# dusk-network/plonk

Measured on AMD Instinct MI355X. Metric: prove() wall-clock (ms) at 2^20 gates, lower is better.
Workload: dtype u32 limbs (Fr 256-bit / Fp 384-bit Montgomery)

## Files before the change

### plonk_amd/__init__.py

```python
from __future__ import annotations

import ctypes
import os
import weakref
from typing import Iterable, Sequence

os.environ.setdefault("HSA_ENABLE_IPC_MODE_LEGACY", "0")

_HERE = os.path.dirname(os.path.abspath(__file__))
LIB_PATH = os.environ.get("PLONK_HIP_LIB") or os.path.join(_HERE, "lib", "libplonk_hip.so")

Q = 0x73EDA753299D7D483339D80809A1D80553BDA402FFFE5BFEFFFFFFFF00000001
P = 0x1A0111EA397FE69A4B1BA7B6434BACD764774B84F38512BF6730D2A0F6B0F6241EABFFFEB153FFFFB9FEFFFFFFFFAAAB
_FR_R = (1 << 256) % Q
_FR_RINV = pow(_FR_R, -1, Q)
_FP_R = (1 << 384) % P
_FP_RINV = pow(_FP_R, -1, P)

PLONK_OK = 0
ERRORS = {
    -1: "PLONK_ERR_ARG", -2: "PLONK_ERR_HIP", -3: "PLONK_ERR_DEGREE (PolynomialDegreeTooLarge)",
    -4: "PLONK_ERR_NO_SRS", -5: "PLONK_ERR_NO_GPU", -6: "PLONK_ERR_UNSAT (CircuitUnsatisfied)",
    -7: "PLONK_ERR_STATE", -8: "PLONK_ERR_BYTES (NotEnoughBytes)", -9: "PLONK_ERR_DATA (InvalidData)",
    -10: "PLONK_ERR_POINT (PointMalformed)", -11: "PLONK_ERR_NOMEM (host allocation failed inside the library)",
# ... 260 lines not shown
    lib.plonk_srs_load_public_parameters.argtypes = [vp, vp, u64, u64, ci, vp, ctypes.POINTER(u64)]
    lib.plonk_lagrange_key.argtypes = [vp, u32, vp]
    lib.plonk_compile.argtypes = [vp, ctypes.POINTER(_CircuitDesc), ctypes.POINTER(vp)]
    lib.plonk_prover_prove_witnesses.argtypes = [vp, vp, u64, vp, vp, u64, vp, vp]
    lib.plonk_prover_to_bytes.argtypes = [vp, vp, u64, ctypes.POINTER(u64)]
    lib.plonk_verifier_to_bytes.argtypes = [vp, vp, u64, vp, u64, vp, u64, ctypes.POINTER(u64)]
    lib.plonk_verifier_from_bytes.argtypes = [vp, vp, u64, ctypes.POINTER(vp)]
    lib.plonk_verifier_destroy.argtypes = [vp]
    lib.plonk_verifier_destroy.restype = None
    lib.plonk_verifier_set_version.argtypes = [vp, ci]
    lib.plonk_verify.argtypes = [vp, vp, vp, u64, u64, vp]
    lib.plonk_verifier_last.argtypes = [vp, vp]
    lib.plonk_test_verify_msm.argtypes = [vp, vp, vp, u64, vp]
    lib.plonk_verify_mixed.argtypes = [vp, u32, vp, vp, vp, u64, u64, vp, vp]
    lib.plonk_test_verify_replay.argtypes = [vp, u32, vp, vp, vp, u64, u64, vp, vp, vp]
    lib.plonk_host_alloc.argtypes = [u64, ctypes.POINTER(vp)]
    lib.plonk_host_free.argtypes = [vp]
    lib.plonk_comm_unique_id.argtypes = [vp]
    lib.plonk_comm_init.argtypes = [vp, vp, ci, ci]
    lib.plonk_comm_selftest.argtypes = [vp]
    lib.plonk_comm_info.argtypes = [vp, ctypes.POINTER(ci), ctypes.POINTER(ci)]
    lib.plonk_comm_destroy.argtypes = [vp]
    lib.plonk_comm_warning.argtypes = [vp, vp, u64]
    lib.plonk_comm_measure_loopback.argtypes = [vp, ci]
    lib.plonk_ctx_create_ex.argtypes = [ctypes.POINTER(vp), ci, ctypes.POINTER(GpuConfig)]
    lib.plonk_ctx_get_config.argtypes = [vp, ctypes.POINTER(GpuConfig)]
    lib.plonk_ctx_set_config.argtypes = [vp, ctypes.POINTER(GpuConfig)]
    lib.plonk_ctx_describe_msm.argtypes = [vp, u64, ci, ci, u32, u64, ctypes.POINTER(_MsmPlan)]
    lib.plonk_ctx_last_msm.argtypes = [vp, ctypes.POINTER(_MsmPlan)]
    lib.plonk_ctx_table_bytes.argtypes = [vp, ctypes.POINTER(u64), ctypes.POINTER(u64)]
# ... 284 lines not shown
        out = ctypes.create_string_buffer(97)
        self._check(self.lib.plonk_test_verify_msm(self.handle, comp, sc, len(points), out))
        return g1_from_raw97(out.raw)

    def _verify_replay(self, items):
        args = _mixed_args(items)
        count = len(items)
        status = (ctypes.c_int32 * count)()
        scalars = ctypes.create_string_buffer(28 * 32 * count)
        digests = ctypes.create_string_buffer(32 * count)
        self._check(self.lib.plonk_test_verify_replay(*args, status, scalars, digests))
        raw = scalars.raw
        return [(int(status[k]), [raw[896 * k + 32 * j:896 * k + 32 * j + 32] for j in range(28)],
                 digests.raw[32 * k:32 * k + 32]) for k in range(count)]

    def alloc(self, nbytes: int) -> DeviceBuffer:
        return DeviceBuffer(self, nbytes)

    def get_config(self) -> "GpuConfig":
        g = GpuConfig()
        self._check(self.lib.plonk_ctx_get_config(self.handle, ctypes.byref(g)))
        return g

    def set_config(self, config: "GpuConfig"):
        self._check(self.lib.plonk_ctx_set_config(self.handle, ctypes.byref(config)))

    def describe_msm(self, m: int, count: int = 1, bit_sum_tail: bool = True, table_rows: int = 0, table_points: int = 0) -> dict:
        p = _MsmPlan()
        self._check(self.lib.plonk_ctx_describe_msm(self.handle, m, count, int(bit_sum_tail), table_rows, table_points, ctypes.byref(p)))
        return p.as_dict()
# ... 685 lines not shown
```

### plonk_amd/csrc/capi.hip

```cpp
#include <chrono>
#include <cstdio>
#include <cstring>
#include <sched.h>
#include <thread>

#include "plonk_internal.hpp"
#include "hostg1.hpp"

namespace plonk {

static thread_local char g_last_error[512] = "";

void set_last_error(const char* what, const char* detail, const char* file, int line) {
  snprintf(g_last_error, sizeof g_last_error, "%s:%d: %s -> %s", file, line, what ? what : "?", detail ? detail : "?");
}

int srs_generate_device(Ctx* c, const Fr& tau, const Fr& g_scalar, uint64_t n, G1Affine* out_dev);

int ctx_refuse_poisoned(const char* api_fn) {
  set_last_error(api_fn, "context unusable: a collective timed out and its stream never drained (comm_sync); destroy the context", __FILE__, __LINE__);
  return PLONK_ERR_STATE;
}

bool ctx_abandon(Ctx* c) {
// ... 171 lines not shown
  if (const int t = env_int("PLONK_COMM_TIMEOUT_MS", 0); t > 0) g.comm_timeout_ms = t;
  if (getenv("PLONK_SIDE_CUS")) g.side_cus = env_int("PLONK_SIDE_CUS", 0);
  g.ksl = env_int("PLONK_MSM_KSL", 0);
  g.prof_fine = env_chr("PLONK_PROF_FINE") == '1';
  g.acc_lds = env_chr("PLONK_MSM_ACC") == 'l';
  if (const char v = env_chr("PLONK_MSM_ORDER")) g.order = v == '1' ? 1 : 0;
  g.tail_serial = env_chr("PLONK_MSM_TAIL") == 's';
  g.bsum_lane = env_chr("PLONK_MSM_BSUM") == 'l';
  g.rc_lane_tree = env_chr("PLONK_MSM_RCTREE") == 'l';
  g.lps = env_int("PLONK_MSM_LPS", 0);
  g.rcwv = env_int("PLONK_MSM_RCWV", 0);
  if (const char v = env_chr("PLONK_MSM_SORT13")) g.sort13 = v == '1' ? 1 : 0;
  g.acc_wg = env_int("PLONK_MSM_ACC_WG", 0);
  g.ntt_direct = env_chr("PLONK_NTT_DIRECT") != '0';
  g.bi_cfg = env_int("PLONK_BI_CFG", -1);
  if (const char v = env_chr("PLONK_SIDE_DEFER")) g.side_defer = v == '1' ? 1 : (v == '2' ? 2 : 0);
  if (const char v = env_chr("PLONK_SIDE_AFTER_ELOG"); v == '2' || v == '3') g.side_after_elog = v - '0';
  if (const char v = env_chr("PLONK_WIRE_POLYS_SIDE")) g.wire_polys_side = v == '1' ? 1 : 0;
  if (env_chr("PLONK_WIRE_BY_COLUMN") == '0') g.wire_by_column = -1;
  if (env_chr("PLONK_WIRE_BY_COLUMN") == '1') g.wire_by_column = 1;
  if (env_chr("PLONK_WIRE_BY_COLUMN") == '2') g.wire_by_column = 2;
  if (getenv("PLONK_HOST_THREADS")) g.host_threads = env_int("PLONK_HOST_THREADS", -1);
  if (g.table_mode != (int)MSM_ROWS_WINDOW && g.table_mode != (int)MSM_ROWS_HALFPOS && g.table_mode != (int)MSM_ROWS_BITPOS) g.table_mode = 0;
  if (g.ntt_elog != 2 && g.ntt_elog != 3) g.ntt_elog = 0;
  if (g.side_cus < 0) g.side_cus = 0;
  if (g.host_threads < 0) {
    cpu_set_t set;
    CPU_ZERO(&set);
    const int cpus = sched_getaffinity(0, sizeof set, &set) == 0 ? CPU_COUNT(&set) : (int)std::thread::hardware_concurrency();
    g.host_threads = cpus >= 8 ? 3 : 0;
// ... 266 lines not shown
  return PLONK_OK;
  });
}

int plonk_ntt_dev(plonk_ctx* ctx, const void* src, void* dst, void* tmp, uint32_t log_n, int inverse,
                  int coset, uint64_t in_len) {
  const char* const api_fn = __func__;
  return plonk::api_guard(api_fn, [&]() -> int {
  if (!ctx || !src || !dst || log_n >= 28) return PLONK_ERR_ARG;
  if (log_n > 10 && !tmp) return PLONK_ERR_ARG;
  CTX_ENTER(ctx->c, api_fn);
  HIP_TRY(hipSetDevice(ctx->c.device));
  prof_begin(&ctx->c, 0);
  int rc = ntt_device(&ctx->c, (const Fr*)src, (Fr*)dst, (Fr*)tmp, log_n, inverse != 0, coset != 0, in_len);
  prof_end(&ctx->c, 0);
  return rc;
  });
}

int plonk_ntt(plonk_ctx* ctx, uint64_t* a, uint32_t log_n, int inverse, int coset, uint64_t in_len) {
  const char* const api_fn = __func__;
  return plonk::api_guard(api_fn, [&]() -> int {
  if (!ctx || !a || log_n >= 28) return PLONK_ERR_ARG;
  Ctx& c = ctx->c;
  CTX_ENTER(c, api_fn);
  HIP_TRY(hipSetDevice(c.device));
  const uint64_t n = 1ull << log_n;
  if (in_len > n) in_len = n;
  int rc = ensure_ntt_staging(&c, n);
  if (rc) return rc;
// ... 299 lines not shown
```

### plonk_amd/csrc/kzg.hip

```cpp
#include <hip/hip_runtime.h>

#include <chrono>
#include <memory>
#include <mutex>
#include <new>
#include <vector>

#include "../../include/plonk_hip.h"
#include "plonk_internal.hpp"
#include "api_guard.hpp"
#include "poly.hpp"
#include "fr29.cuh"
#include "hostg1.hpp"
#include "hostpairing.hpp"
#include "verify_core.hpp"
#include "kzg_core.hpp"

#define PTRY_K(expr) do { int _rc = (expr); if (_rc) return _rc; } while (0)
#define KZG_FAIL(code, msg) return (plonk::set_last_error(api_fn, msg, __FILE__, __LINE__), code)

namespace plonk { struct KzgKey; }
struct plonk_kzg_key {
  plonk::KzgKey* k;
  plonk_ctx* ctx;
// ... 148 lines not shown
  for (uint32_t i = 0; i < n; ++i) L = desc[i].len > L ? desc[i].len : L;
  if (L > c.srs_n) return PLONK_ERR_DEGREE;
  identity48(witness48);
  if (!L) {
    for (uint64_t i = 0; i < 4 * count; ++i) evaluations[i] = 0;
    if (commitments) for (uint32_t i = 0; i < n; ++i) identity48(commitments + 48ull * i);
    return PLONK_OK;
  }
  PTRY_K(msm_reserve(&c, L));
  PTRY_K(w.need(KzgWork::DESC, sizeof(KzgDesc) * n));
  PTRY_K(w.need(KzgWork::VPOW, sizeof(Fr29Slot) * n));
  PTRY_K(w.need(KzgWork::EVALS, sizeof(Fr) * n));
  PTRY_K(w.need(KzgWork::PARTIAL, sizeof(Fr) * KZG_GROUP * kzg_fold_waves(L)));
  PTRY_K(w.need(KzgWork::FOLD, sizeof(Fr) * (L + 1)));
  PTRY_K(w.need(KzgWork::SCRATCH, sizeof(Fr) * (L + 1)));
  PTRY_K(w.need(KzgWork::TOTALS, sizeof(Fr) * (L / 2048 + 2)));
  prof_begin(&c, 12);
  PTRY_K(poly_kzg_powers(&c, w.p[KzgWork::VPOW], n, v));
  HIP_TRY(hipMemsetAsync(w.p[KzgWork::EVALS], 0, sizeof(Fr) * n, c.stream));
  bool started = false;
  if (resident) {
    for (uint32_t first = 0; first < n; first += KZG_GROUP) {
      const uint32_t cnt = n - first < KZG_GROUP ? n - first : KZG_GROUP;
      uint64_t glen = 0;
      for (uint32_t i = 0; i < cnt; ++i) glen = desc[first + i].len > glen ? desc[first + i].len : glen;
      if (glen) PTRY_K(fold_group(&c, w, first, cnt, glen, L, &started, z));
    }
    prof_end(&c, 12);
    if (commitments) PTRY_K(commit_polys(&c, desc.data(), n, commitments));
  } else {
    const uint64_t S = L > KZG_STAGE_MIN ? L : KZG_STAGE_MIN;
// ... 299 lines not shown
```

### plonk_amd/csrc/plonk_internal.hpp

```cpp
#pragma once
#include <hip/hip_runtime.h>
#include <stdint.h>

#include <map>
#include <mutex>
#include <set>
#include <vector>

#include "../../include/plonk_hip.h"
#include "api_guard.hpp"
#include "curve.cuh"
#include "msm_recode.cuh"

#define HIP_TRY(expr)                                                    \
  do {                                                                   \
    hipError_t _e = (expr);                                              \
    if (_e != hipSuccess) {                                              \
      plonk::set_last_error(#expr, hipGetErrorString(_e), __FILE__, __LINE__); \
      return PLONK_ERR_HIP;                                              \
    }                                                                    \
  } while (0)

namespace plonk {

// ... 112 lines not shown
  int comm_timeout_ms = 120000;
  int side_cus = 0;
  int ksl = 0;
  bool prof_fine = false;
  bool acc_lds = false;
  int order = -1;
  bool tail_serial = false;
  bool bsum_lane = false;
  bool rc_lane_tree = false;
  int lps = 0;
  int rcwv = 0;
  int sort13 = -1;
  int acc_wg = 0;
  bool ntt_direct = true;
  int bi_cfg = -1;
  int side_defer = -1;
  int wire_by_column = 0;
  int wire_polys_side = -1;
  int side_after_elog = 0;
  int host_threads = -1;
};

struct plonk_msm_plan_internal {
  uint32_t table_rows = 0, bucket_bits = 0, digit_width = 0, slice_entries = 0, ordered_lanes = 0, wide_words = 0, flags = 0;
  uint64_t terms = 0;
  const char* kernel = "";
};

struct Ctx {
  int device = 0;
// ... 129 lines not shown
```

### plonk_amd/csrc/poly.hip

```cpp
#include <cstdlib>

#include "plonk_internal.hpp"
#include "fr29.cuh"
#include "fp_safegcd.cuh"
#include "poly.hpp"

namespace plonk {

__device__ __forceinline__ Fr ldf(const Fr* p) {
  const uint4* q = reinterpret_cast<const uint4*>(p);
  uint4 a = q[0], b = q[1];
  Fr r;
  r.l[0] = a.x; r.l[1] = a.y; r.l[2] = a.z; r.l[3] = a.w;
  r.l[4] = b.x; r.l[5] = b.y; r.l[6] = b.z; r.l[7] = b.w;
  return r;
}
__device__ __forceinline__ void stf(Fr* p, const Fr& v) {
  uint4* q = reinterpret_cast<uint4*>(p);
  q[0] = make_uint4(v.l[0], v.l[1], v.l[2], v.l[3]);
  q[1] = make_uint4(v.l[4], v.l[5], v.l[6], v.l[7]);
}
__device__ __forceinline__ Fr small(uint32_t v, const Fr& one) {
  Fr acc = Fr::zero();
  Fr p = one;
// ... 63 lines not shown

__global__ void scatter_pi_kernel(Fr* dense, const uint64_t* idx, const Fr* val, uint64_t count) {
  const uint64_t i = (uint64_t)blockIdx.x * blockDim.x + threadIdx.x;
  if (i < count) stf(dense + idx[i], ldf(val + i));
}

struct Tw {
  uint32_t w[9];
};
__device__ __forceinline__ Fr29 tw29(const Tw& t) {
  Fr29 r;
#pragma unroll
  for (int i = 0; i < 9; ++i) r.l[i] = t.w[i];
  return r;
}
static Tw tw_of(const Fr& x) {
  const Fr29 t = Fr29::twiddle_from_fr(x);
  Tw r;
  for (int i = 0; i < 9; ++i) r.w[i] = t.l[i];
  return r;
}
static Tw tw_plain(const Fr& x) {
  const Fr29 t = Fr29::from_fr(x);
  Tw r;
  for (int i = 0; i < 9; ++i) r.w[i] = t.l[i];
  return r;
}
__device__ __forceinline__ Fr29 ld29_(const Fr* p) { return Fr29::from_fr(ldf(p)); }
__device__ __forceinline__ Fr29 pow_tw(const Fr29& xt, uint64_t e, const Fr29& one_t) {
  Fr29 acc = one_t;
// ... 329 lines not shown
  Tw gamma_t;
  Tw bk_t[4];
  Tw b32_t;
  Tw one_t;
};
__device__ __forceinline__ Fr29 ld_slot(const void* base, uint64_t idx) {
  const uint4* q = reinterpret_cast<const uint4*>(reinterpret_cast<const Fr29Slot*>(base) + idx);
  const uint4 a = q[0], b = q[1];
  const uint32_t c = reinterpret_cast<const Fr29Slot*>(base)[idx].w[8];
  Fr29 r;
  r.l[0] = a.x; r.l[1] = a.y; r.l[2] = a.z; r.l[3] = a.w;
  r.l[4] = b.x; r.l[5] = b.y; r.l[6] = b.z; r.l[7] = b.w;
  r.l[8] = c;
  return r;
}
__global__ void __launch_bounds__(128) perm_terms_kernel(PermArgs a, PermConst k) {
  const uint64_t j0 = (uint64_t)blockIdx.x * blockDim.x + threadIdx.x;
  if (j0 >= a.count) return;
  const uint64_t i = a.first + j0;
  if (i == 0) {
    const Fr one = tw29(k.one_t).to_fr();
    stf(a.num, one);
    stf(a.den, one);
    return;
  }
  const uint64_t r = i - 1;
  Fr29 root = ld_slot(a.tw_lo29, r & ((1ull << a.lobits) - 1));
  if (a.use_hi) root = Fr29::mul(root, ld_slot(a.tw_hi29, r >> a.lobits));
  const Fr29 conv = tw29(k.conv), gamma_t = tw29(k.gamma_t), b32 = tw29(k.b32_t);
  Fr29 num, den;
#pragma unroll
  for (int j = 0; j < 4; ++j) {
    const Fr29 wg = Fr29::add_csub(Fr29::mul(ld29_(a.wires[j] + r), conv), gamma_t);
    const Fr29 nf = Fr29::add_csub(wg, Fr29::mul(root, tw29(k.bk_t[j])));
    const Fr29 df = Fr29::add_csub(wg, Fr29::mul(ld29_(a.sigma[j] + r), b32));
    num = j ? Fr29::mul(num, nf) : nf;
    den = j ? Fr29::mul(den, df) : df;
  }
  stf(a.num + i, num.to_fr());
  stf(a.den + i, den.to_fr());
}
__global__ void mul_arrays_kernel(Fr* __restrict__ a, const Fr* __restrict__ b, uint64_t n, int* zero_flag) {
  const uint64_t i = (uint64_t)blockIdx.x * blockDim.x + threadIdx.x;
  if (i >= n) return;
  const Fr y = ldf(b + i);
  if (zero_flag && y.is_zero()) *zero_flag = 1;
  stf(a + i, Fr29::mul(ld29_(a + i), Fr29::from_fr(y)).to_fr());
}

__device__ __forceinline__ Fr delta4(const Fr& f, const Fr& one) {
  const Fr two = one.dbl();
  return f * (f - one) * (f - two) * (f - two - one);
}

__device__ __forceinline__ Fr29 ld29(const Fr* p) { return Fr29::from_fr(ldf(p)); }
// ... 259 lines not shown
      const Fr29 w = tw29(a.pw[b]);
      p = started ? Fr29::mul(p, w) : w;
      started = true;
    }
  }
  const Fr29 step = tw29(a.pw[6]);
#pragma unroll 1
  for (int k = 0; k < E; ++k) {
    const uint64_t i = first + 64ull * k;
    if (i >= n) break;
    stf(dst + i, Fr29::mul(Fr29::add_csub(ld29_(src + i + src_off), add), p).to_fr());
    if (E > 1) p = Fr29::mul(p, step);
  }
}

__global__ void fold_kernel(const Fr* __restrict__ src, Fr* __restrict__ dst, uint64_t n, uint32_t extra, Fr c) {
  const uint64_t i = (uint64_t)blockIdx.x * blockDim.x + threadIdx.x;
  if (i >= n) return;
  Fr v = ldf(src + i);
  if (i < extra) v = v + c * ldf(src + n + i);
  stf(dst + i, v);
}

__global__ void shard_pack_kernel(ShardPackArgs a) {
  const uint64_t i = (uint64_t)blockIdx.x * blockDim.x + threadIdx.x;
  const uint32_t k = blockIdx.y, peer = blockIdx.z;
  if (i >= a.stride) return;
  const Fr* F = a.F[k];
  Fr v = Fr::zero();
  if (i < a.per) {
// ... 120 lines not shown
  PermConst k;
  k.conv = tw_of(Fr::from_u64(32));
  k.gamma_t = tw_of(a.gamma);
  for (int j = 0; j < 4; ++j) k.bk_t[j] = tw_of(a.beta * a.ks[j]);
  k.b32_t = tw_of(a.beta * Fr::from_u64(32));
  k.one_t = tw_of(Fr::one());
  PermArgs r = a;
  if (r.count == 0) { r.first = 0; r.count = a.n; }
  if (r.first + r.count > a.n) return (plonk::set_last_error("invalid argument", __func__, __FILE__, __LINE__), PLONK_ERR_ARG);
  hipLaunchKernelGGL(perm_terms_kernel, grid1(r.count, 128), dim3(128), 0, c->stream, r, k);
  HIP_TRY(hipGetLastError());
  return PLONK_OK;
}
int poly_mul_arrays(Ctx* c, Fr* a, const Fr* b, uint64_t n, int* zero_flag) {
  hipLaunchKernelGGL(mul_arrays_kernel, grid1(n, 256), dim3(256), 0, c->stream, a, b, n, zero_flag);
  HIP_TRY(hipGetLastError());
  return PLONK_OK;
}
int poly_quotient(Ctx* c, const QuotientArgs& q) {
  prof_begin(c, 3);
  WidgetConst wc{};
  if (q.has[QS_RANGE] | q.has[QS_LOGIC] | q.has[QS_FIXED] | q.has[QS_VAR]) {
    wc.conv = tw_of(Fr::from_u64(32));
    wc.one_r = tw_plain(Fr::one());
    wc.c1 = tw_of(Fr::one()); wc.c3 = tw_of(Fr::from_u64(3)); wc.c9 = tw_of(Fr::from_u64(9));
    wc.c18 = tw_of(Fr::from_u64(18)); wc.c81 = tw_of(Fr::from_u64(81)); wc.c83 = tw_of(Fr::from_u64(83));
    wc.ed = tw_of(q.edwards_d);
    Fr k = q.range_ch.sqr(), w = q.range_ch;
    for (int j = 0; j < 4; ++j) { wc.rg[j] = tw_of(w); w = w * k; }
    k = q.logic_ch.sqr();
// ... 113 lines not shown
  uint32_t nbits = 7;
  while (nbits < MP_BITS && (emax >> nbits)) ++nbits;
  Fr29 p = Fr29::twiddle_from_fr(x);
  for (uint32_t b = 0; b < nbits; ++b) {
    for (int i = 0; i < 9; ++i) a.pw[b].w[i] = p.l[i];
    p = Fr29::mul(p, p);
  }
  a.one_t = tw_of(Fr::one());
  a.addend = addend;
  a.nbits = nbits;
  a.zero_at = zero_at;
  if (n <= (1ull << 17)) hipLaunchKernelGGL(mul_powers_kernel<1>, grid1(n, 256), dim3(256), 0, c->stream, src, dst, n, a, src_off, exp_off);
  else if (n <= (1ull << 19)) hipLaunchKernelGGL(mul_powers_kernel<4>, grid1((n + 3) / 4 + 64, 256), dim3(256), 0, c->stream, src, dst, n, a, src_off, exp_off);
  else hipLaunchKernelGGL(mul_powers_kernel<16>, grid1((n + 15) / 16 + 64, 256), dim3(256), 0, c->stream, src, dst, n, a, src_off, exp_off);
}
int poly_ruffini(Ctx* c, const Fr* src, Fr* dst, uint64_t len, const Fr& z, const Fr& zinv, Fr* scratch, Fr* totals) {
  launch_mul_powers(c, src, scratch, len, z, 0, 0);
  int rc = scan_suffix_sum(c, scratch, len, totals);
  if (rc) return rc;
  launch_mul_powers(c, scratch, dst, len - 1, zinv, 1, 1, Fr::zero(), len - 1);
  HIP_TRY(hipGetLastError());
  return PLONK_OK;
}

__device__ __forceinline__ void st_slot(void* base, uint64_t idx, const Fr29& v) {
  uint32_t* w = reinterpret_cast<Fr29Slot*>(base)[idx].w;
#pragma unroll
  for (int i = 0; i < 9; ++i) w[i] = v.l[i];
  w[9] = 0; w[10] = 0; w[11] = 0;
}
__global__ void __launch_bounds__(256) kzg_powers_kernel(void* __restrict__ tab, uint32_t count, Tw xt, Tw one_t) {
// ... 157 lines not shown
```

### plonk_amd/csrc/poly.hpp

```cpp
#pragma once
#include "plonk_internal.hpp"

namespace plonk {

enum { QS_M = 0, QS_L, QS_R, QS_O, QS_F, QS_C, QS_ARITH, QS_RANGE, QS_LOGIC, QS_FIXED, QS_VAR, QS_COUNT };

struct BlindArgs {
  int count;
  Fr b[3];
};
struct SplitArgs {
  Fr b[3];
  uint64_t len4;
};
struct PermArgs {
  uint64_t n;
  uint64_t first = 0, count = 0;
  const Fr* wires[4];
  const Fr* sigma[4];
  Fr beta, gamma;
  Fr ks[4];
  const void* tw_lo29;
  const void* tw_hi29;
  uint32_t lobits;
// ... 107 lines not shown

void prof_begin(Ctx* c, int slot);
void prof_end(Ctx* c, int slot);
void prof_host_add(Ctx* c, int slot, double ms);

int poly_fill_zero(Ctx* c, Fr* p, uint64_t n);
int poly_blind(Ctx* c, Fr* coeffs, uint64_t n, const BlindArgs& a);
int poly_split_t(Ctx* c, Fr* t, uint64_t n, uint64_t np, Fr* out, const SplitArgs& a);
int poly_trimmed_len(Ctx* c, const Fr* p, uint64_t n, unsigned long long* out_dev);
int poly_scatter_pi(Ctx* c, Fr* dense, const uint64_t* idx, const Fr* val, uint64_t count);
int poly_sigma_evals(Ctx* c, const uint32_t* map_dev, const Fr* roots, Fr* out, uint64_t n, uint64_t stride, const SigmaArgs& a);
int poly_gather_wires(Ctx* c, const uint32_t* idx_dev, const Fr* values, Fr* wires, uint64_t constraints, uint64_t n);
int poly_batch_inverse(Ctx* c, Fr* v, uint64_t n, bool twiddle_form = false);
int poly_perm_terms(Ctx* c, const PermArgs& a);
int poly_mul_arrays(Ctx* c, Fr* a, const Fr* b, uint64_t n, int* zero_flag);
int poly_quotient(Ctx* c, const QuotientArgs& q);
int poly_dealias(Ctx* c, Fr* t, uint64_t nq, const Fr low[7], const Fr& g_inv);
int poly_l1(Ctx* c, const Fr* linear, Fr* l1, uint64_t n8, const L1Args& a);
int poly_scale_array(Ctx* c, Fr* v, uint64_t n, const Fr& s);
int poly_from_mont(Ctx* c, const Fr* src, Fr* dst, uint64_t n);
void quotient_const(const Fr& c, int shift, uint32_t out[9]);
void quotient_data(const Fr& c, uint32_t out[9]);
int poly_eval(Ctx* c, EvalArgs& a, int count, uint64_t max_len, Fr* out_dev);
int poly_lincomb(Ctx* c, const LinCombArgs& a);
int poly_ruffini(Ctx* c, const Fr* src, Fr* dst, uint64_t len, const Fr& z, const Fr& zinv, Fr* scratch, Fr* totals);
int scan_prefix_product(Ctx* c, Fr* data, uint64_t n, Fr* totals);
uint32_t scan_prefix_blocks(uint64_t n);
int scan_prefix_product_local(Ctx* c, Fr* data, uint64_t n, Fr* totals);
int scan_prefix_product_apply(Ctx* c, Fr* data, uint64_t n, const Fr* totals, const Fr& carry_twiddle);
int scan_suffix_sum(Ctx* c, Fr* data, uint64_t n, Fr* totals);
// ... 3 lines not shown
```

### plonk_amd/csrc/prover.hip

```cpp
#include <cstdlib>
#include <cstring>
#include <random>
#include <string>
#include <vector>

#include "poly.hpp"
#include "transcript.hpp"
#include <chrono>

#include "hostg1.hpp"
#include "finish_pool.hpp"
#include "widgets.hpp"
#include "permutation.hpp"
#include "diagnose.hpp"
#include "composer.hpp"

static_assert(plonk::DQ_M == plonk::QS_M && plonk::DQ_ARITH == plonk::QS_ARITH && plonk::DQ_VAR == plonk::QS_VAR &&
              plonk::DQ_COUNT == plonk::QS_COUNT, "diagnose_core.hpp selector ids");
static_assert(plonk::WQS_RANGE == plonk::QS_RANGE && plonk::WQS_LOGIC == plonk::QS_LOGIC && plonk::WQS_FIXED == plonk::QS_FIXED &&
              plonk::WQS_VAR == plonk::QS_VAR && plonk::WQS_COUNT == plonk::QS_COUNT, "widgets.hpp selector ids");

namespace plonk {

struct Prover {
// ... 833 lines not shown

  const Fr beta = tr.challenge_scalar("beta");
  tr.append_scalar("beta", beta);
  const Fr gamma = tr.challenge_scalar("gamma");
  {
    prof_begin(c, 4);
    PermArgs pa;
    pa.n = n;
    for (int k = 0; k < 4; ++k) { pa.wires[k] = wires_dev + k * n; pa.sigma[k] = p->sigma_n + k * n; }
    pa.beta = beta; pa.gamma = gamma;
    pa.ks[0] = Fr::one(); pa.ks[1] = fr_small(7); pa.ks[2] = fr_small(13); pa.ks[3] = fr_small(17);
    pa.tw_lo29 = tbn->tw_lo29; pa.tw_hi29 = tbn->tw_hi29; pa.lobits = L < 13 ? L : 13; pa.use_hi = L > 13;
    pa.num = p->scratch; pa.den = p->scratch + np;
    gap.launching();
    HIP_TRY(hipMemsetAsync(p->flag_dev, 0, sizeof(int), c->stream));
    PTRY(poly_perm_terms(c, pa));
    PTRY(poly_batch_inverse(c, pa.den, n, true));
    PTRY(poly_mul_arrays(c, pa.num, pa.den, n, p->flag_dev));
    PTRY(scan_prefix_product(c, pa.num, n, p->totals));
    if (!z_from_evals) {
      PTRY(ntt_device(c, pa.num, p->zpoly, p->tmp8, L, true, false, n));
      BlindArgs ba;
      ba.count = 3;
      ba.b[0] = bl[8]; ba.b[1] = bl[9]; ba.b[2] = bl[10];
      PTRY(poly_fill_zero(c, p->zpoly + n, np - n));
      PTRY(poly_blind(c, p->zpoly, n, ba));
    }
    prof_end(c, 4);
  }
  auto z_polynomial = [&](Fr* ntt_tmp) -> int {
    PTRY(ntt_device(c, p->scratch, p->zpoly, ntt_tmp, L, true, false, n));
    BlindArgs ba;
    ba.count = 3;
    ba.b[0] = bl[8]; ba.b[1] = bl[9]; ba.b[2] = bl[10];
// ... 387 lines not shown
  const Fr gamma = tr.challenge_scalar("gamma");
  {
    prof_begin(c, 4);
    PermArgs pa;
    pa.n = n;
    for (int k = 0; k < 4; ++k) { pa.wires[k] = wires_dev + k * n; pa.sigma[k] = p->sigma_n + k * n; }
    pa.beta = beta; pa.gamma = gamma;
    pa.ks[0] = Fr::one(); pa.ks[1] = fr_small(7); pa.ks[2] = fr_small(13); pa.ks[3] = fr_small(17);
    pa.tw_lo29 = tbn->tw_lo29; pa.tw_hi29 = tbn->tw_hi29; pa.lobits = L < 13 ? L : 13; pa.use_hi = L > 13;
    pa.num = p->scratch; pa.den = p->scratch + np;
    gap.launching();
    HIP_TRY(hipMemsetAsync(p->flag_dev, 0, sizeof(int), c->stream));
    const int shard_z_env = c->cfg.shard_z > 0 ? 1 : (c->cfg.shard_z < 0 ? 0 : -1);
    const bool shard_z = (shard_z_env >= 0 ? shard_z_env == 1 : (L >= 19 && W >= 4)) && n % W == 0 && n / W >= 2;
    if (!shard_z) {
      PTRY(poly_perm_terms(c, pa));
      PTRY(poly_batch_inverse(c, pa.den, n, true));
      PTRY(poly_mul_arrays(c, pa.num, pa.den, n, p->flag_dev));
      PTRY(scan_prefix_product(c, pa.num, n, p->totals));
    } else {
      const uint64_t cnt = n / W, first = cnt * (uint64_t)p->rank;
      pa.first = first; pa.count = cnt;
      PTRY(poly_perm_terms(c, pa));
      PTRY(poly_batch_inverse(c, pa.den + first, cnt, true));
      PTRY(poly_mul_arrays(c, pa.num + first, pa.den + first, cnt, p->flag_dev));
      PTRY(scan_prefix_product_local(c, pa.num + first, cnt, p->totals));
      struct { Fr total; int flag; int pad[7]; } mine, *all;
      static_assert(sizeof(mine) == 64, "exchange record");
      memset(&mine, 0, sizeof mine);
      HIP_TRY(hipMemcpyAsync(p->ev_host, p->totals + (scan_prefix_blocks(cnt) - 1), sizeof(Fr), hipMemcpyDeviceToHost, c->stream));
      HIP_TRY(hipMemcpyAsync(p->flag_host, p->flag_dev, sizeof(int), hipMemcpyDeviceToHost, c->stream));
      const auto t_before = HostGap::clock::now();
      PTRY(comm_sync(c, c->stream));
      gap.synced(t_before);
// ... 870 lines not shown
```

Before: 31.24.

## Fuse permutation grand-product and Ruffini division into block-scan kernels

Replaces the four-kernel permutation Z pipeline (perm terms, batch inverse, multiply, prefix product) with a single block kernel. It computes the terms, inverts the denominators per block with a shared inversion, and runs the block prefix product, followed by the usual totals and apply passes. Ruffini division is likewise fused: the power multiply and suffix sum happen in one block kernel, and the apply kernel rescales by inverse powers computed on the fly. The aim is to cut kernel launches and global memory round trips for the num/den and scratch arrays, at the cost of more register pressure and a per-block field inversion. Test entry points are added, and the KZG totals buffer is enlarged to match the new block size.

```diff
diff --git a/plonk_amd/__init__.py b/plonk_amd/__init__.py
--- a/plonk_amd/__init__.py
+++ b/plonk_amd/__init__.py
@@ -298,6 +298,9 @@
     lib.plonk_test_verify_msm.argtypes = [vp, vp, vp, u64, vp]
     lib.plonk_verify_mixed.argtypes = [vp, u32, vp, vp, vp, u64, u64, vp, vp]
     lib.plonk_test_verify_replay.argtypes = [vp, u32, vp, vp, vp, u64, u64, vp, vp, vp]
+    if hasattr(lib, "plonk_test_perm_z"):
+        lib.plonk_test_perm_z.argtypes = [vp, vp, vp, u32, vp, vp, vp, vp, ctypes.POINTER(ci)]
+        lib.plonk_test_ruffini.argtypes = [vp, vp, vp, u64, vp, vp, vp]
     lib.plonk_host_alloc.argtypes = [u64, ctypes.POINTER(vp)]
     lib.plonk_host_free.argtypes = [vp]
     lib.plonk_comm_unique_id.argtypes = [vp]
@@ -612,6 +615,16 @@
         return [(int(status[k]), [raw[896 * k + 32 * j:896 * k + 32 * j + 32] for j in range(28)],
                  digests.raw[32 * k:32 * k + 32]) for k in range(count)]
 
+    def _perm_z(self, wires: int, sigma: int, log_n: int, beta: int, gamma: int, z_out: int, scratch: int) -> int:
+        flag = ctypes.c_int(0)
+        self._check(self.lib.plonk_test_perm_z(self.handle, wires, sigma, log_n, fr_to_bytes_mont([beta]), fr_to_bytes_mont([gamma]),
+                                               z_out, scratch, ctypes.byref(flag)))
+        return flag.value
+
+    def _ruffini(self, src: int, dst: int, length: int, z: int, scratch: int):
+        self._check(self.lib.plonk_test_ruffini(self.handle, src, dst, length, fr_to_bytes_mont([z]),
+                                                fr_to_bytes_mont([pow(z, -1, Q)]), scratch))
+
     def alloc(self, nbytes: int) -> DeviceBuffer:
         return DeviceBuffer(self, nbytes)
 
diff --git a/plonk_amd/csrc/capi.hip b/plonk_amd/csrc/capi.hip
--- a/plonk_amd/csrc/capi.hip
+++ b/plonk_amd/csrc/capi.hip
@@ -6,6 +6,7 @@
 
 #include "plonk_internal.hpp"
 #include "hostg1.hpp"
+#include "poly.hpp"
 
 namespace plonk {
 
@@ -209,6 +210,8 @@
   g.acc_wg = env_int("PLONK_MSM_ACC_WG", 0);
   g.ntt_direct = env_chr("PLONK_NTT_DIRECT") != '0';
   g.bi_cfg = env_int("PLONK_BI_CFG", -1);
+  g.perm_fused = env_chr("PLONK_PERM_FUSED") != '0';
+  g.ruffini_fused = env_chr("PLONK_RUFFINI_FUSED") != '0';
   if (const char v = env_chr("PLONK_SIDE_DEFER")) g.side_defer = v == '1' ? 1 : (v == '2' ? 2 : 0);
   if (const char v = env_chr("PLONK_SIDE_AFTER_ELOG"); v == '2' || v == '3') g.side_after_elog = v - '0';
   if (const char v = env_chr("PLONK_WIRE_POLYS_SIDE")) g.wire_polys_side = v == '1' ? 1 : 0;
@@ -505,6 +508,63 @@
   prof_begin(&ctx->c, 0);
   int rc = ntt_device(&ctx->c, (const Fr*)src, (Fr*)dst, (Fr*)tmp, log_n, inverse != 0, coset != 0, in_len);
   prof_end(&ctx->c, 0);
+  return rc;
+  });
+}
+
+int plonk_test_perm_z(plonk_ctx* ctx, const void* wires, const void* sigma, uint32_t log_n, const uint32_t* beta,
+                      const uint32_t* gamma, void* z_out, void* scratch, int* flag_out) {
+  const char* const api_fn = __func__;
+  return plonk::api_guard(api_fn, [&]() -> int {
+  if (!ctx || !wires || !sigma || !beta || !gamma || !z_out || !scratch || !flag_out || log_n < 1 || log_n > 24)
+    return (plonk::set_last_error("invalid argument", api_fn, __FILE__, __LINE__), PLONK_ERR_ARG);
+  Ctx& c = ctx->c;
+  CTX_ENTER(c, api_fn);
+  HIP_TRY(hipSetDevice(c.device));
+  const uint64_t n = 1ull << log_n;
+  NttTables* tb;
+  int rc = ntt_tables(&c, log_n, false, &tb);
+  if (rc) return rc;
+  Fr* totals = nullptr;
+  HIP_TRY(hipMalloc((void**)&totals, sizeof(Fr) * (256 * 64 + 1) + sizeof(int)));
+  int* flag_dev = reinterpret_cast<int*>(totals + 256 * 64 + 1);
+  PermArgs pa;
+  pa.n = n;
+  for (int k = 0; k < 4; ++k) { pa.wires[k] = (const Fr*)wires + k * n; pa.sigma[k] = (const Fr*)sigma + k * n; }
+  memcpy(pa.beta.l, beta, 32);
+  memcpy(pa.gamma.l, gamma, 32);
+  pa.ks[0] = Fr::one(); pa.ks[1] = Fr::from_u64(7); pa.ks[2] = Fr::from_u64(13); pa.ks[3] = Fr::from_u64(17);
+  pa.tw_lo29 = tb->tw_lo29; pa.tw_hi29 = tb->tw_hi29; pa.lobits = log_n < 13 ? log_n : 13; pa.use_hi = log_n > 13;
+  pa.num = (Fr*)z_out; pa.den = (Fr*)scratch;
+  hipError_t e = hipMemsetAsync(flag_dev, 0, sizeof(int), c.stream);
+  if (e == hipSuccess) rc = poly_perm_z(&c, pa, totals, flag_dev);
+  if (e == hipSuccess && rc == PLONK_OK) e = hipMemcpyAsync(flag_out, flag_dev, sizeof(int), hipMemcpyDeviceToHost, c.stream);
+  const hipError_t e2 = hipStreamSynchronize(c.stream);
+  (void)hipFree(totals);
+  HIP_TRY(e);
+  HIP_TRY(e2);
+  if (rc == PLONK_OK && *flag_out)
+    return (plonk::set_last_error("invalid argument", "zero denominator in the permutation grand product", __FILE__, __LINE__), PLONK_ERR_ARG);
+  return rc;
+  });
+}
+int plonk_test_ruffini(plonk_ctx* ctx, const void* src, void* dst, uint64_t len, const uint32_t* z, const uint32_t* zinv, void* scratch) {
+  const char* const api_fn = __func__;
+  return plonk::api_guard(api_fn, [&]() -> int {
+  if (!ctx || !src || !dst || !z || !zinv || !scratch || len < 1 || len > (1ull << 24))
+    return (plonk::set_last_error("invalid argument", api_fn, __FILE__, __LINE__), PLONK_ERR_ARG);
+  Ctx& c = ctx->c;
+  CTX_ENTER(c, api_fn);
+  HIP_TRY(hipSetDevice(c.device));
+  Fr zz, zi;
+  memcpy(zz.l, z, 32);
+  memcpy(zi.l, zinv, 32);
+  Fr* totals = nullptr;
+  HIP_TRY(hipMalloc((void**)&totals, sizeof(Fr) * (256 * 64 + 1)));
+  const int rc = poly_ruffini(&c, (const Fr*)src, (Fr*)dst, len, zz, zi, (Fr*)scratch, totals);
+  const hipError_t e = hipStreamSynchronize(c.stream);
+  (void)hipFree(totals);
+  HIP_TRY(e);
   return rc;
   });
 }
diff --git a/plonk_amd/csrc/kzg.hip b/plonk_amd/csrc/kzg.hip
--- a/plonk_amd/csrc/kzg.hip
+++ b/plonk_amd/csrc/kzg.hip
@@ -186,7 +186,7 @@
   PTRY_K(w.need(KzgWork::PARTIAL, sizeof(Fr) * KZG_GROUP * kzg_fold_waves(L)));
   PTRY_K(w.need(KzgWork::FOLD, sizeof(Fr) * (L + 1)));
   PTRY_K(w.need(KzgWork::SCRATCH, sizeof(Fr) * (L + 1)));
-  PTRY_K(w.need(KzgWork::TOTALS, sizeof(Fr) * (L / 2048 + 2)));
+  PTRY_K(w.need(KzgWork::TOTALS, sizeof(Fr) * (L / 512 + 2)));
   prof_begin(&c, 12);
   PTRY_K(poly_kzg_powers(&c, w.p[KzgWork::VPOW], n, v));
   HIP_TRY(hipMemsetAsync(w.p[KzgWork::EVALS], 0, sizeof(Fr) * n, c.stream));
diff --git a/plonk_amd/csrc/plonk_internal.hpp b/plonk_amd/csrc/plonk_internal.hpp
--- a/plonk_amd/csrc/plonk_internal.hpp
+++ b/plonk_amd/csrc/plonk_internal.hpp
@@ -150,6 +150,8 @@
   int acc_wg = 0;
   bool ntt_direct = true;
   int bi_cfg = -1;
+  bool perm_fused = true;
+  bool ruffini_fused = true;
   int side_defer = -1;
   int wire_by_column = 0;
   int wire_polys_side = -1;
diff --git a/plonk_amd/csrc/poly.hip b/plonk_amd/csrc/poly.hip
--- a/plonk_amd/csrc/poly.hip
+++ b/plonk_amd/csrc/poly.hip
@@ -1,4 +1,6 @@
 #include <cstdlib>
+#include <type_traits>
+#include <utility>
 
 #include "plonk_internal.hpp"
 #include "fr29.cuh"
@@ -101,6 +103,10 @@
   for (int i = 0; i < 9; ++i) r.l[i] = t.w[i];
   return r;
 }
+template <typename F, int... I>
+__device__ __forceinline__ void static_for_seq(F&& f, std::integer_sequence<int, I...>) { (f(std::integral_constant<int, I>{}), ...); }
+template <int N, typename F>
+__device__ __forceinline__ void static_for(F&& f) { static_for_seq(f, std::make_integer_sequence<int, N>{}); }
 static Tw tw_of(const Fr& x) {
   const Fr29 t = Fr29::twiddle_from_fr(x);
   Tw r;
@@ -460,6 +466,19 @@
   r.l[8] = c;
   return r;
 }
+__device__ __forceinline__ void perm_term(const PermArgs& a, const PermConst& k, uint64_t r, Fr29& num, Fr29& den) {
+  Fr29 root = ld_slot(a.tw_lo29, r & ((1ull << a.lobits) - 1));
+  if (a.use_hi) root = Fr29::mul(root, ld_slot(a.tw_hi29, r >> a.lobits));
+  const Fr29 conv = tw29(k.conv), gamma_t = tw29(k.gamma_t), b32 = tw29(k.b32_t);
+#pragma unroll
+  for (int j = 0; j < 4; ++j) {
+    const Fr29 wg = Fr29::add_csub(Fr29::mul(ld29_(a.wires[j] + r), conv), gamma_t);
+    const Fr29 nf = Fr29::add_csub(wg, Fr29::mul(root, tw29(k.bk_t[j])));
+    const Fr29 df = Fr29::add_csub(wg, Fr29::mul(ld29_(a.sigma[j] + r), b32));
+    num = j ? Fr29::mul(num, nf) : nf;
+    den = j ? Fr29::mul(den, df) : df;
+  }
+}
 __global__ void __launch_bounds__(128) perm_terms_kernel(PermArgs a, PermConst k) {
   const uint64_t j0 = (uint64_t)blockIdx.x * blockDim.x + threadIdx.x;
   if (j0 >= a.count) return;
@@ -470,21 +489,86 @@
     stf(a.den, one);
     return;
   }
-  const uint64_t r = i - 1;
-  Fr29 root = ld_slot(a.tw_lo29, r & ((1ull << a.lobits) - 1));
-  if (a.use_hi) root = Fr29::mul(root, ld_slot(a.tw_hi29, r >> a.lobits));
-  const Fr29 conv = tw29(k.conv), gamma_t = tw29(k.gamma_t), b32 = tw29(k.b32_t);
   Fr29 num, den;
-#pragma unroll
-  for (int j = 0; j < 4; ++j) {
-    const Fr29 wg = Fr29::add_csub(Fr29::mul(ld29_(a.wires[j] + r), conv), gamma_t);
-    const Fr29 nf = Fr29::add_csub(wg, Fr29::mul(root, tw29(k.bk_t[j])));
-    const Fr29 df = Fr29::add_csub(wg, Fr29::mul(ld29_(a.sigma[j] + r), b32));
-    num = j ? Fr29::mul(num, nf) : nf;
-    den = j ? Fr29::mul(den, df) : df;
-  }
+  perm_term(a, k, i - 1, num, den);
   stf(a.num + i, num.to_fr());
   stf(a.den + i, den.to_fr());
+}
+
+template <bool FINAL, int E>
+__global__ void __launch_bounds__(SCAN_T) perm_ratio_scan_block_kernel(PermArgs a, PermConst k, PScanArgs s, Fr* __restrict__ totals,
+                                                                       int* zero_flag) {
+  __shared__ uint32_t shp[9][SCAN_T], shs[9][SCAN_T], shinv[9];
+  const int t = threadIdx.x;
+  const uint64_t base = (uint64_t)blockIdx.x * (SCAN_T * E) + (uint64_t)t * E;
+  const Fr29 one_t = tw29(k.one_t);
+  Fr29 num[E], den[E], pre[E];
+  Fr29 acc = one_t;
+  uint32_t nz = 0;
+  static_for<E>([&](auto ic) __attribute__((always_inline)) {
+    constexpr int e = decltype(ic)::value;
+    pre[e] = acc;
+    num[e] = one_t;
+    den[e] = one_t;
+    const uint64_t i = base + e;
+    if (i < a.n) {
+      if (i) perm_term(a, k, i - 1, num[e], den[e]);
+      if (den[e].to_fr().is_zero()) {
+        *zero_flag = 1;
+      } else {
+        nz |= 1u << e;
+        acc = Fr29::mul(acc, den[e]);
+      }
+    }
+  });
+  Fr29 pfx = acc, sfx = acc;
+  for (int d = 1; d < SCAN_T; d <<= 1) {
+    ps_put(shp, t, pfx);
+    ps_put(shs, t, sfx);
+    __syncthreads();
+    if (t >= d) pfx = Fr29::mul(pfx, ps_get(shp, t - d));
+    if (t + d < SCAN_T) sfx = Fr29::mul(sfx, ps_get(shs, t + d));
+    __syncthreads();
+  }
+  ps_put(shp, t, pfx);
+  ps_put(shs, t, sfx);
+  __syncthreads();
+  if (t == 0) {
+    const Fr29 r = fr29_inv_gcd_tw(sfx);
+#pragma unroll
+    for (int i = 0; i < 9; ++i) shinv[i] = r.l[i];
+  }
+  __syncthreads();
+  Fr29 outer;
+#pragma unroll
+  for (int i = 0; i < 9; ++i) outer.l[i] = shinv[i];
+  if (t > 0) outer = Fr29::mul(outer, ps_get(shp, t - 1));
+  if (t + 1 < SCAN_T) outer = Fr29::mul(outer, ps_get(shs, t + 1));
+  Fr29 suf = outer;
+  static_for<E>([&](auto ic) __attribute__((always_inline)) {
+    constexpr int e = E - 1 - decltype(ic)::value;
+    if ((nz >> e) & 1) {
+      num[e] = Fr29::mul(num[e], Fr29::mul(suf, pre[e]));
+      suf = Fr29::mul(suf, den[e]);
+    } else if (base + e < a.n) {
+      num[e] = Fr29::zero();
+    }
+  });
+  acc = one_t;
+  static_for<E>([&](auto ic) __attribute__((always_inline)) {
+    constexpr int e = decltype(ic)::value;
+    if (base + e < a.n) acc = Fr29::mul(acc, num[e]);
+    num[e] = acc;
+  });
+  __syncthreads();
+  Fr29 tot;
+  const Fr29 excl = ps_lanes(acc, shp, t, one_t, &tot);
+  if (t == 0) stf(totals + blockIdx.x, tot.to_fr());
+  const Fr29 post = FINAL ? Fr29::mul(excl, tw29(s.one_r)) : excl;
+  static_for<E>([&](auto ic) __attribute__((always_inline)) {
+    constexpr int e = decltype(ic)::value;
+    if (base + e < a.n) stf(a.num + base + e, Fr29::mul(post, num[e]).to_fr());
+  });
 }
 __global__ void mul_arrays_kernel(Fr* __restrict__ a, const Fr* __restrict__ b, uint64_t n, int* zero_flag) {
   const uint64_t i = (uint64_t)blockIdx.x * blockDim.x + threadIdx.x;
@@ -774,6 +858,81 @@
   }
 }
 
+struct RufArgs {
+  Tw pw[MP_BITS];
+  Tw step;
+  Tw one_t;
+  uint32_t nbits;
+};
+__device__ __forceinline__ Fr29 ruf_pow(const RufArgs& a, uint64_t e) {
+  Fr29 p = tw29(a.one_t);
+  bool started = false;
+#pragma unroll 1
+  for (uint32_t b = 0; b < a.nbits; ++b) {
+    if ((e >> b) & 1) {
+      const Fr29 w = tw29(a.pw[b]);
+      p = started ? Fr29::mul(p, w) : w;
+      started = true;
+    }
+  }
+  return p;
+}
+template <int E>
+__global__ void __launch_bounds__(SCAN_T) ruffini_block_kernel(const Fr* src, Fr* scratch, uint64_t n, Fr* __restrict__ totals, RufArgs a) {
+  __shared__ uint32_t sh[9][SCAN_T];
+  const int t = threadIdx.x;
+  const uint64_t base = (uint64_t)blockIdx.x * (SCAN_T * E) + (uint64_t)t * E;
+  Fr29 v[E];
+  Fr29 acc = Fr29::zero();
+  Fr29 p = tw29(a.one_t);
+  if (base < n) p = ruf_pow(a, n - 1 - base);
+  const Fr29 step = tw29(a.step);
+  static_for<E>([&](auto ic) __attribute__((always_inline)) {
+    constexpr int e = decltype(ic)::value;
+    const uint64_t li = base + e;
+    if (li < n) {
+      acc = Fr29::add_csub(acc, Fr29::mul(ld29_(src + (n - 1 - li)), p));
+      if (e + 1 < E) p = Fr29::mul(p, step);
+    }
+    v[e] = acc;
+  });
+  for (int d = 1; d < SCAN_T; d <<= 1) {
+    ps_put(sh, t, acc);
+    __syncthreads();
+    if (t >= d) acc = Fr29::add_csub(ps_get(sh, t - d), acc);
+    __syncthreads();
+  }
+  ps_put(sh, t, acc);
+  __syncthreads();
+  const Fr29 excl = t ? ps_get(sh, t - 1) : Fr29::zero();
+  if (t == SCAN_T - 1) stf(totals + blockIdx.x, acc.to_fr());
+  static_for<E>([&](auto ic) __attribute__((always_inline)) {
+    constexpr int e = decltype(ic)::value;
+    const uint64_t li = base + e;
+    if (li < n) stf(scratch + (n - 1 - li), Fr29::add_csub(excl, v[e]).to_fr());
+  });
+}
+template <int E>
+__global__ void __launch_bounds__(SCAN_T) ruffini_apply_kernel(Fr* scratch, Fr* dst, uint64_t n, const Fr* __restrict__ totals, RufArgs a) {
+  if (blockIdx.x == 0 && threadIdx.x == 0) stf(dst + (n - 1), Fr::zero());
+  const uint64_t base = (uint64_t)blockIdx.x * (SCAN_T * E) + (uint64_t)threadIdx.x * E;
+  if (base >= n) return;
+  const Fr29 off = blockIdx.x ? ld29_(totals + blockIdx.x - 1) : Fr29::zero();
+  Fr29 p = ruf_pow(a, n - 1 - base);
+  const Fr29 step = tw29(a.step);
+#pragma unroll
+  for (int e = 0; e < E; ++e) {
+    const uint64_t li = base + e;
+    if (li < n) {
+      const uint64_t gi = n - 1 - li;
+      const Fr29 s = Fr29::add_csub(ld29_(scratch + gi), off);
+      if (gi) stf(dst + (gi - 1), Fr29::mul(s, p).to_fr());
+      else if (blockIdx.x) stf(scratch, s.to_fr());
+      if (e + 1 < E) p = Fr29::mul(p, step);
+    }
+  }
+}
+
 __global__ void fold_kernel(const Fr* __restrict__ src, Fr* __restrict__ dst, uint64_t n, uint32_t extra, Fr c) {
   const uint64_t i = (uint64_t)blockIdx.x * blockDim.x + threadIdx.x;
   if (i >= n) return;
@@ -924,6 +1083,44 @@
 }
 int poly_mul_arrays(Ctx* c, Fr* a, const Fr* b, uint64_t n, int* zero_flag) {
   hipLaunchKernelGGL(mul_arrays_kernel, grid1(n, 256), dim3(256), 0, c->stream, a, b, n, zero_flag);
+  HIP_TRY(hipGetLastError());
+  return PLONK_OK;
+}
+static inline int perm_fused_e(uint64_t n) { return n <= (1ull << 17) ? 2 : 4; }
+int poly_perm_z(Ctx* c, const PermArgs& a, Fr* totals, int* zero_flag) {
+  const uint64_t n = a.n;
+  const int e = perm_fused_e(n);
+  const uint64_t blk = (uint64_t)SCAN_T * e;
+  const uint64_t nb64 = (n + blk - 1) / blk;
+  if (a.count != 0 || n == 0 || !zero_flag) return (plonk::set_last_error("invalid argument", __func__, __FILE__, __LINE__), PLONK_ERR_ARG);
+  if (!c->cfg.perm_fused || nb64 > (uint64_t)SCAN_T * SCAN_MAXPER) {
+    int rc = poly_perm_terms(c, a);
+    if (rc == PLONK_OK) rc = poly_batch_inverse(c, a.den, n, true);
+    if (rc == PLONK_OK) rc = poly_mul_arrays(c, a.num, a.den, n, zero_flag);
+    if (rc == PLONK_OK) rc = scan_prefix_product(c, a.num, n, totals);
+    return rc;
+  }
+  const uint32_t nb = (uint32_t)nb64;
+  PermConst k;
+  k.conv = tw_of(Fr::from_u64(32));
+  k.gamma_t = tw_of(a.gamma);
+  for (int j = 0; j < 4; ++j) k.bk_t[j] = tw_of(a.beta * a.ks[j]);
+  k.b32_t = tw_of(a.beta * Fr::from_u64(32));
+  k.one_t = tw_of(Fr::one());
+  PScanArgs s{};
+  s.one_t = k.one_t;
+  s.one_r = tw_plain(Fr::one());
+#define PRS_LAUNCH(FINAL, E) \
+  hipLaunchKernelGGL((perm_ratio_scan_block_kernel<FINAL, E>), dim3(nb), dim3(SCAN_T), 0, c->stream, a, k, s, totals, zero_flag)
+  if (nb == 1) {
+    if (e == 2) PRS_LAUNCH(true, 2); else PRS_LAUNCH(true, 4);
+  } else {
+    if (e == 2) PRS_LAUNCH(false, 2); else PRS_LAUNCH(false, 4);
+    hipLaunchKernelGGL(pscan_totals_kernel, dim3(1), dim3(SCAN_T), 0, c->stream, totals, nb, (nb + SCAN_T - 1) / SCAN_T, s);
+    if (e == 2) hipLaunchKernelGGL(pscan_apply_kernel<2>, dim3(nb), dim3(SCAN_T), 0, c->stream, a.num, n, totals, s);
+    else hipLaunchKernelGGL(pscan_apply_kernel<4>, dim3(nb), dim3(SCAN_T), 0, c->stream, a.num, n, totals, s);
+  }
+#undef PRS_LAUNCH
   HIP_TRY(hipGetLastError());
   return PLONK_OK;
 }
@@ -1067,7 +1264,35 @@
   else if (n <= (1ull << 19)) hipLaunchKernelGGL(mul_powers_kernel<4>, grid1((n + 3) / 4 + 64, 256), dim3(256), 0, c->stream, src, dst, n, a, src_off, exp_off);
   else hipLaunchKernelGGL(mul_powers_kernel<16>, grid1((n + 15) / 16 + 64, 256), dim3(256), 0, c->stream, src, dst, n, a, src_off, exp_off);
 }
+static void ruf_args(RufArgs& a, const Fr& x, const Fr& xinv, uint64_t emax) {
+  uint32_t nbits = 1;
+  while (nbits < MP_BITS && (emax >> nbits)) ++nbits;
+  Fr29 p = Fr29::twiddle_from_fr(x);
+  for (uint32_t b = 0; b < nbits; ++b) {
+    for (int i = 0; i < 9; ++i) a.pw[b].w[i] = p.l[i];
+    p = Fr29::mul(p, p);
+  }
+  a.step = tw_of(xinv);
+  a.one_t = tw_of(Fr::one());
+  a.nbits = nbits;
+}
+template <int E>
+static void ruffini_fused_launch(Ctx* c, const Fr* src, Fr* dst, uint64_t len, const RufArgs& az, const RufArgs& ai, Fr* scratch, Fr* totals) {
+  const uint32_t nb = (uint32_t)((len + SCAN_T * E - 1) / (SCAN_T * E));
+  hipLaunchKernelGGL(ruffini_block_kernel<E>, dim3(nb), dim3(SCAN_T), 0, c->stream, src, scratch, len, totals, az);
+  if (nb > 1) hipLaunchKernelGGL((scan_totals_kernel<false>), dim3(1), dim3(SCAN_T), 0, c->stream, totals, nb, (nb + SCAN_T - 1) / SCAN_T);
+  hipLaunchKernelGGL(ruffini_apply_kernel<E>, dim3(nb), dim3(SCAN_T), 0, c->stream, scratch, dst, len, (const Fr*)totals, ai);
+}
 int poly_ruffini(Ctx* c, const Fr* src, Fr* dst, uint64_t len, const Fr& z, const Fr& zinv, Fr* scratch, Fr* totals) {
+  if (c->cfg.ruffini_fused && len >= 2 && len <= (uint64_t)SCAN_BLOCK * SCAN_T * SCAN_MAXPER && src != scratch && dst != scratch) {
+    RufArgs az{}, ai{};
+    ruf_args(az, z, zinv, len - 1);
+    ruf_args(ai, zinv, z, len - 1);
+    if (len <= (1ull << 17)) ruffini_fused_launch<2>(c, src, dst, len, az, ai, scratch, totals);
+    else ruffini_fused_launch<8>(c, src, dst, len, az, ai, scratch, totals);
+    HIP_TRY(hipGetLastError());
+    return PLONK_OK;
+  }
   launch_mul_powers(c, src, scratch, len, z, 0, 0);
   int rc = scan_suffix_sum(c, scratch, len, totals);
   if (rc) return rc;
diff --git a/plonk_amd/csrc/poly.hpp b/plonk_amd/csrc/poly.hpp
--- a/plonk_amd/csrc/poly.hpp
+++ b/plonk_amd/csrc/poly.hpp
@@ -145,6 +145,7 @@
 int poly_batch_inverse(Ctx* c, Fr* v, uint64_t n, bool twiddle_form = false);
 int poly_perm_terms(Ctx* c, const PermArgs& a);
 int poly_mul_arrays(Ctx* c, Fr* a, const Fr* b, uint64_t n, int* zero_flag);
+int poly_perm_z(Ctx* c, const PermArgs& a, Fr* totals, int* zero_flag);
 int poly_quotient(Ctx* c, const QuotientArgs& q);
 int poly_dealias(Ctx* c, Fr* t, uint64_t nq, const Fr low[7], const Fr& g_inv);
 int poly_l1(Ctx* c, const Fr* linear, Fr* l1, uint64_t n8, const L1Args& a);
diff --git a/plonk_amd/csrc/prover.hip b/plonk_amd/csrc/prover.hip
--- a/plonk_amd/csrc/prover.hip
+++ b/plonk_amd/csrc/prover.hip
@@ -871,10 +871,7 @@
     pa.num = p->scratch; pa.den = p->scratch + np;
     gap.launching();
     HIP_TRY(hipMemsetAsync(p->flag_dev, 0, sizeof(int), c->stream));
-    PTRY(poly_perm_terms(c, pa));
-    PTRY(poly_batch_inverse(c, pa.den, n, true));
-    PTRY(poly_mul_arrays(c, pa.num, pa.den, n, p->flag_dev));
-    PTRY(scan_prefix_product(c, pa.num, n, p->totals));
+    PTRY(poly_perm_z(c, pa, p->totals, p->flag_dev));
     if (!z_from_evals) {
       PTRY(ntt_device(c, pa.num, p->zpoly, p->tmp8, L, true, false, n));
       BlindArgs ba;
@@ -1292,10 +1289,7 @@
     const int shard_z_env = c->cfg.shard_z > 0 ? 1 : (c->cfg.shard_z < 0 ? 0 : -1);
     const bool shard_z = (shard_z_env >= 0 ? shard_z_env == 1 : (L >= 19 && W >= 4)) && n % W == 0 && n / W >= 2;
     if (!shard_z) {
-      PTRY(poly_perm_terms(c, pa));
-      PTRY(poly_batch_inverse(c, pa.den, n, true));
-      PTRY(poly_mul_arrays(c, pa.num, pa.den, n, p->flag_dev));
-      PTRY(scan_prefix_product(c, pa.num, n, p->totals));
+      PTRY(poly_perm_z(c, pa, p->totals, p->flag_dev));
     } else {
       const uint64_t cnt = n / W, first = cnt * (uint64_t)p->rank;
       pa.first = first; pa.count = cnt;
```

New measurement: 31.14 (median of 5 runs). About the same (-0.3%).
